# nathancunn/ParticleMDI.jl

Hardware: NVIDIA B200
Metric: particle*cluster*feature evals/sec (dense count P*N*sum_k D_k per observation step) (higher is better)
Workload: dtype f64

## Files before the change

particlemdi.jl_b200/csrc/pmdi_cuda.cu:

```cuda
#include "../../include/pmdi_cuda.h"

#include <cuda_runtime.h>
#include <dlfcn.h>

#include <algorithm>
#include <chrono>
#include <cmath>
#include <cstdio>
#include <cstring>
#include <cstdlib>
#include <map>
#include <queue>
#include <string>
#include <vector>

#include "aux_kernels.cuh"
#include "sweep_kernel.cuh"
#include "pool_kernel.cuh"
#include "spec_kernel.cuh"
#include "summary_kernels.cuh"

#include "pmdi_embedded.inc"

#ifndef __CUDA_ARCH__
// ... 61 lines not shown

struct Dataset {
  bool bound = false;
  int type = -1, D = 0, Dp = 0, J = 0, Lmax = 0, FB = PMDI_FB;
  int user = -1, uW = 0;
  int slot = 0;
  DevBuf<double> ust;
  long long max_arg = 0;
  std::vector<uint8_t> flag;
  std::vector<double> nlevels;
  bool rc_dirty = true;
  DevBuf<unsigned char> x, xq;
  bool xq_dirty = true;
  DevBuf<uint8_t> d_flag;
  DevBuf<double> rc, d_nlevels;
  DevBuf<double> mu, lamn, sum, beta, part, aux;
  DevBuf<uint32_t> cnt;
  DevBuf<long long> S;
  DevBuf<int> n;
  int cap = 0, wpf = 1, fpw = 4;
  DevBuf<unsigned long long> cw;
  DevBuf<int> p_refcnt, p_chosen, p_dst, p_neval, p_live, p_free, p_rowmap, p_ctr;
  DevBuf<double> p_lp;
  DevBuf<RowInfo> p_info;
  DevBuf<int> p_mark;
  void release() {
    x.release(); xq.release(); d_flag.release(); rc.release(); d_nlevels.release();
    mu.release(); lamn.release(); sum.release(); beta.release(); part.release(); aux.release();
    cnt.release(); S.release(); n.release(); cw.release(); ust.release();
    p_refcnt.release(); p_chosen.release(); p_dst.release(); p_neval.release(); p_live.release();
    p_free.release(); p_rowmap.release(); p_ctr.release(); p_lp.release();
    p_info.release(); p_mark.release();
  }
};

}

struct pmdi_ctx {
  int K = 0, N = 0, P = 0, device = 0;
  long long n = 0;
  cudaStream_t stream = nullptr;
  bool own_stream = false;
  int n_sm = 0, G = 0, GP = 0;
  int sm_budget = 0;
  pmdi_group* group = nullptr;
  std::vector<Dataset> ds;
  bool layout_dirty = true;
  unsigned char* arena = nullptr;
  size_t arena_bytes = 0;
  int rank = 0, R = 1, Ps = 0;
  int engine = 1;
  int engine_req = PMDI_ENGINE_AUTO;
  int obs_ring = PMDI_OBS_RING;
  unsigned long long wd_ns = 10000000000ull;
  long long peer_delta[8] = {0, 0, 0, 0, 0, 0, 0, 0};
  void* peer_base[8] = {nullptr, nullptr, nullptr, nullptr, nullptr, nullptr, nullptr, nullptr};
  std::vector<int> cta_off, cta_units;
  int max_units = 0, sm_x_bytes = 0, lf_T = 0, lf_want = 0, item_cap = 0, Jmax = 0;
  bool assigned = false;
  size_t dyn_smem = 0;
  std::vector<double> lf_host;
  DevBuf<double> lf_dev;
  DevBuf<int> d_cta_off, d_cta_units;
  DevBuf<double> Pi, l1phi, tape_alloc, tape_resamp, tape_shuffle, tape_select;
  DevBuf<long long> s_in, s_out, d_pstar, cluster_n, counters;
  DevBuf<int> order, slot_of, anc_log, ev_of_step, members, mem_off, cur_at, plan_out, err;
  DevBuf<int> sc_j, sc_anc0, sc_a, sc_b, sc_c, sc_d;
  DevBuf<double> lw, lw_out, sc_w, sc_pp, sc_u, inc, lp_empty, ess_part;
  DevBuf<int> logical_of;
  DevBuf<uint8_t> lab, alloc_log;
  DevBuf<int2> copies;
  DevBuf<unsigned> bar;
  DevBuf<unsigned long long> rows_eval, rows_ref, phase_ns, trace;
  DevBuf<long long> label_counts, pair_agree, contingency;
  DevBuf<unsigned> psm;
  DevBuf<long long> psm_s;
  long long psm_samples = 0;
  DevBuf<double> rank_part;
  DevBuf<int4> pull_jobs;
  DevBuf<int> pull_map;
  bool pull_map_init = false;
  DevBuf<unsigned char> dec;
  DevBuf<int4> glist, elist;
  DevBuf<int> gcnt;
  DevBuf<unsigned long long> rows_spec, rows_add;
  DevBuf<double> dbg_lp, dbg_lw, scratch_d;
  DevBuf<int> dbg_alloc, dbg_anc, scratch_i, wd_state;
  DevBuf<uint8_t> scratch_u8;
  SweepParams sp;
  bool uploaded = false, ran = false;
  cudaLibrary_t jit_lib = nullptr;
  std::string jit_key;
  std::vector<UserType> jit_types;
  bool has_user = false;
  unsigned step_seq = 0;
  unsigned long long sweep_seq = 1;
  DevBuf<unsigned long long> bar_state;
  bool bar_state_init = false;
  unsigned sweep_flags = 0;
  cudaEvent_t ev0 = nullptr, ev1 = nullptr, ev2 = nullptr, ev3 = nullptr;
  DevBuf<unsigned char> inblk, outblk;
  unsigned char *h_in = nullptr, *h_out = nullptr;
  size_t in_bytes = 0, out_bytes = 0, out_head = 0;
  struct { size_t s_in, Pi, l1phi, order; } ioff;
  struct { size_t err, counters, rows_eval, rows_ref, rows_spec, rows_add, pstar, label_counts, pair_agree,
           contingency, lw_out, s_out, phase, cluster_n; } ooff;
  cudaEvent_t ev_h2d = nullptr;
};

namespace {

int round_up(int v, int m) { return (v + m - 1) / m * m; }

void fill_dsdev(pmdi_ctx* c, int k, DsDev& d) {
  Dataset& s = c->ds[k];
  std::memset(&d, 0, sizeof(d));
  d.type = s.type; d.D = s.D; d.Dp = s.Dp; d.J = s.J; d.Lmax = s.type == T_USER ? s.slot : s.Lmax; d.FB = s.FB;
  int nflag = 0;
  for (int q = 0; q < s.D; ++q) nflag += s.flag[q] ? 1 : 0;
  d.nflag = nflag;
  d.all_on = (nflag == s.D && s.D == s.Dp) ? 1 : 0;
  if (s.type == T_GAUSSIAN && nflag == s.D) d.all_on = 1;
  d.x = s.x.p; d.flag = s.d_flag.p; d.rc = s.rc.p;
  d.xstage = (s.type != T_GAUSSIAN && s.type != T_USER && nflag != s.D) ? (const void*)s.xq.p : (const void*)s.x.p;
  d.mu = s.mu.p; d.lamn = s.lamn.p; d.sum = s.sum.p; d.beta = s.beta.p;
  d.uW = s.type == T_USER ? (user_types()[s.user].elem_kind == PMDI_F64 ? s.uW : -s.uW) : 0;
  d.ust = s.ust.p;
  d.cnt = s.cnt.p; d.S = s.S.p; d.part = c->engine ? nullptr : s.part.p; d.aux = s.aux.p; d.n = s.n.p;
}

void fill_pooldev(pmdi_ctx* c, int k, PoolDev& d) {
  Dataset& s = c->ds[k];
  std::memset(&d, 0, sizeof(d));
  d.cap = s.cap; d.wpf = s.wpf; d.fpw = s.fpw;
  d.refcnt = s.p_refcnt.p; d.chosen = s.p_chosen.p; d.dst = s.p_dst.p; d.n_eval = s.p_neval.p;
  d.live = s.p_live.p; d.freelist = s.p_free.p; d.rowmap = s.p_rowmap.p; d.ctr = s.p_ctr.p; d.cw = s.cw.p;
  d.lp = s.p_lp.p; d.info = s.p_info.p; d.mark = s.p_mark.p;
}

int build_rc(pmdi_ctx* c, int k) {
  Dataset& s = c->ds[k];
  const long long n = c->n;
  std::vector<double> rc(n + 1);
  int nflag = 0;
  for (int q = 0; q < s.D; ++q) nflag += s.flag[q] ? 1 : 0;
  if (s.type == T_USER) {
    std::fill(rc.begin(), rc.end(), 0.0);
  } else if (s.type == T_GAUSSIAN) {
    for (long long i = 0; i <= n; ++i) {
      const double nn = (double)i;
      rc[i] = nflag * (std::log(1.0 / std::sqrt(M_PI)) + std::lgamma(0.5 * nn + 1.0) -
                       std::lgamma(0.5 * nn + 0.5));
    }
  } else if (s.type == T_CATEGORICAL) {
    std::map<double, long long> hist;
    for (int q = 0; q < s.D; ++q)
      if (s.flag[q]) hist[s.nlevels[q]] += 1;
    for (long long i = 0; i <= n; ++i) {
      double acc = 0.0;
      for (auto& kv : hist) acc += (double)kv.second * std::log(kv.first + (double)i);
      rc[i] = -acc;
    }
  } else {
    for (long long i = 0; i <= n; ++i) rc[i] = nflag * std::log((double)i + 1.0);
  }
  CK(s.rc.ensure(n + 1));
// ... 467 lines not shown
  if (tag == PMDI_ALL_USER_TYPES) {
    for (int u = 0; u < (int)user_types().size(); ++u) users.push_back(u);
    if (users.empty()) return fail(1, "pmdi_cluster_type_check: no cluster type registered");
  } else {
    const int user = tag - USER_TAG0;
    if (user < 0 || user >= (int)user_types().size()) return fail(1, "pmdi_cluster_type_check: unknown type tag");
    users.push_back(user);
  }
  const char* eng = getenv("PMDI_ENGINE");
  const std::string* cubin = nullptr;
  return jit_compile(registered(users), eng && std::string(eng) == "spec" ? 2 : 1, cubin);
}

int pmdi_group_type_check(const int32_t* tags, int32_t n) {
  if (!tags) return fail(1, "pmdi_group_type_check: tags is NULL");
  if (n < 1 || n > PMDI_MAX_K) return fail(1, "pmdi_group_type_check: need 1 <= n <= 8 cluster types");
  std::vector<int> users;
  for (int i = 0; i < n; ++i) {
    const int user = tags[i] - USER_TAG0;
    if (user < 0 || user >= (int)user_types().size())
      return fail(1, "pmdi_group_type_check: tags[" + std::to_string(i) + "] is not a registered user type");
    users.push_back(user);
  }
  const std::string* cubin = nullptr;
  return jit_compile(registered(users), JIT_SPEC_GROUP, cubin);
}

int pmdi_ctx_create(pmdi_ctx** out, int32_t K, int64_t n_obs, int32_t N, int32_t particles,
                    int32_t device) {
  if (!out) return fail(1, "pmdi_ctx_create: out is NULL");
  *out = nullptr;
  if (K < 1 || K > PMDI_MAX_K) return fail(1, "pmdi_ctx_create: need 1 <= K <= 8 datasets");
  if (!(N > 1 && (int64_t)N <= n_obs)) return fail(1, "pmdi_ctx_create: need 1 < N <= n_obs");
  if (N > PMDI_MAX_N) return fail(1, "pmdi_ctx_create: N > 256 is not supported");
  if (particles <= 1) return fail(1, "pmdi_ctx_create: need particles > 1");
  if (n_obs > 0x7fffffff / 2) return fail(1, "pmdi_ctx_create: n_obs too large");
  if (pmdi_device_count() <= device || device < 0)
    return fail(2, "pmdi_ctx_create: no CUDA device " + std::to_string(device) +
                       " (libpmdi_cuda has no CPU fallback)");
  CK(cudaSetDevice(device));
  cudaDeviceProp prop;
  CK(cudaGetDeviceProperties(&prop, device));
  if (prop.major < 10)
    return fail(2, "pmdi_ctx_create: built for sm_100a (B200); found compute capability " +
                       std::to_string(prop.major) + "." + std::to_string(prop.minor));
  int coop = 0;
  CK(cudaDeviceGetAttribute(&coop, cudaDevAttrCooperativeLaunch, device));
  if (!coop) return fail(2, "pmdi_ctx_create: device lacks cooperative launch");
  pmdi_ctx* c = new pmdi_ctx();
  c->K = K; c->n = n_obs; c->N = N; c->P = particles; c->device = device;
  c->n_sm = prop.multiProcessorCount;
  c->G = c->n_sm;
  c->sm_budget = c->n_sm;
  c->ds.resize(K);
  std::memset(&c->sp, 0, sizeof(c->sp));
  cudaError_t e = cudaStreamCreateWithFlags(&c->stream, cudaStreamNonBlocking);
  if (e != cudaSuccess) { delete c; return fail(100 + (int)e, "cudaStreamCreate failed"); }
  c->own_stream = true;
  cudaEventCreate(&c->ev0); cudaEventCreate(&c->ev1); cudaEventCreate(&c->ev2); cudaEventCreate(&c->ev3);
  *out = c;
  return 0;
}

static void group_detach(pmdi_ctx* c);

int pmdi_ctx_destroy(pmdi_ctx* c) {
  if (!c) return 0;
  cudaSetDevice(c->device);
  if (c->group) group_detach(c);
  cudaStreamSynchronize(c->stream);
  for (auto& d : c->ds) d.release();
  DevBuf<double>* dd[] = {&c->lf_dev, &c->Pi, &c->l1phi, &c->tape_alloc, &c->tape_resamp, &c->tape_shuffle,
                          &c->tape_select, &c->lw, &c->lw_out, &c->sc_w, &c->sc_pp, &c->sc_u, &c->dbg_lp,
                          &c->dbg_lw, &c->scratch_d, &c->inc, &c->lp_empty, &c->ess_part};
  for (auto* b : dd) b->release();
  DevBuf<int>* di[] = {&c->d_cta_off, &c->d_cta_units, &c->order, &c->slot_of, &c->anc_log, &c->ev_of_step,
                       &c->members, &c->mem_off, &c->cur_at, &c->plan_out, &c->err, &c->sc_j, &c->sc_anc0,
                       &c->sc_a, &c->sc_b, &c->sc_c, &c->sc_d, &c->dbg_alloc, &c->dbg_anc, &c->scratch_i, &c->logical_of};
  for (auto* b : di) b->release();
  DevBuf<long long>* dl[] = {&c->s_in, &c->s_out, &c->d_pstar, &c->cluster_n, &c->counters};
  for (auto* b : dl) b->release();
  c->lab.release(); c->alloc_log.release(); c->copies.release(); c->bar.release();
  c->rows_eval.release(); c->phase_ns.release(); c->scratch_u8.release();
  c->dec.release(); c->rows_spec.release(); c->rows_add.release(); c->bar_state.release(); c->glist.release(); c->elist.release(); c->gcnt.release();
  c->rows_ref.release(); c->trace.release(); c->wd_state.release(); c->pull_jobs.release(); c->pull_map.release(); c->rank_part.release();
  c->label_counts.release(); c->pair_agree.release(); c->contingency.release(); c->psm.release(); c->psm_s.release();
  for (int r = 0; r < c->R; ++r)
    if (r != c->rank && c->peer_base[r]) cudaIpcCloseMemHandle(c->peer_base[r]);
  c->inblk.release(); c->outblk.release();
  if (c->h_in) cudaFreeHost(c->h_in);
  if (c->h_out) cudaFreeHost(c->h_out);
  if (c->ev_h2d) cudaEventDestroy(c->ev_h2d);
  if (c->arena) cudaFree(c->arena);
  if (c->jit_lib) cudaLibraryUnload(c->jit_lib);
  if (c->ev0) { cudaEventDestroy(c->ev0); cudaEventDestroy(c->ev1); cudaEventDestroy(c->ev2); cudaEventDestroy(c->ev3); }
  if (c->own_stream && c->stream) cudaStreamDestroy(c->stream);
  delete c;
  return 0;
}

int pmdi_ctx_set_engine(pmdi_ctx* c, int32_t engine) {
  if (!c) return fail(1, "pmdi_ctx_set_engine: NULL context");
  if (engine != PMDI_ENGINE_AUTO && engine != PMDI_ENGINE_POOL && engine != PMDI_ENGINE_SPEC)
    return fail(1, "pmdi_ctx_set_engine: engine is PMDI_ENGINE_AUTO (-1), PMDI_ENGINE_POOL (1) or PMDI_ENGINE_SPEC (2)");
  if (c->arena)
    return fail(1, "pmdi_ctx_set_engine: the context has already been prepared for the " + engine_name(c->engine) +
                       " engine (first upload, sweep, feature or cluster-eval call), and its memory layout depends on "
                       "the engine: choose the engine before that");
  c->engine_req = engine;
  return 0;
}

int pmdi_ctx_set_stream(pmdi_ctx* c, void* s) {
  if (!c) return fail(1, "NULL context");
  if (c->own_stream && c->stream) cudaStreamDestroy(c->stream);
  c->stream = (cudaStream_t)s;
  c->own_stream = false;
  return 0;
}
void* pmdi_ctx_get_stream(pmdi_ctx* c) { return c ? (void*)c->stream : nullptr; }

int pmdi_set_dataset(pmdi_ctx* c, int32_t k, int32_t type_tag, int32_t elem_kind, const void* data,
                     int64_t n_obs, int64_t D, int64_t ld) {
  if (!c) return fail(1, "NULL context");
  if (k < 0 || k >= c->K) return fail(1, "pmdi_set_dataset: k out of range");
  if (n_obs != c->n) return fail(1, "pmdi_set_dataset: datasets must have n_obs rows (src/pmdi.jl:52)");
  if (D < 1 || D > 8192) return fail(1, "pmdi_set_dataset: need 1 <= D <= 8192 features per dataset");
  if (ld < n_obs) return fail(1, "pmdi_set_dataset: ld < n_obs");
  const int user = type_tag >= USER_TAG0 ? type_tag - USER_TAG0 : -1;
  if (user >= (int)user_types().size() || (user < 0 && (type_tag < 0 || type_tag > 2)))
    return fail(1, "pmdi_set_dataset: unknown cluster type tag");
  if (user >= 0) {
    if (elem_kind != user_types()[user].elem_kind)
      return fail(1, "pmdi_set_dataset: cluster type '" + user_types()[user].name + "' was registered for the other element kind");
  } else if ((type_tag == PMDI_GAUSSIAN) != (elem_kind == PMDI_F64)) {
    return fail(1, "pmdi_set_dataset: Gaussian needs PMDI_F64 data, Categorical/NegBinom need PMDI_I64");
  }
  CK(cudaSetDevice(c->device));
  Dataset& s = c->ds[k];
  s.release();
  s.type = user >= 0 ? T_USER : type_tag; s.user = user; s.D = (int)D; s.Dp = round_up((int)D, PMDI_WF);
  s.J = (s.Dp + PMDI_FB - 1) / PMDI_FB;
  s.Lmax = 0; s.max_arg = 0;
  const long long n = c->n;
  const int Dp = s.Dp;
  s.flag.assign(Dp, 0);
  for (int q = 0; q < s.D; ++q) s.flag[q] = 1;
  if (user >= 0) {
    const int w = user_words_guess(user_types()[user].src);
    if (w < 1 || w > 8) return fail(1, "pmdi_set_dataset: the user type needs `static constexpr int WORDS = 1..8;`");
    s.uW = w;
  }
  if (elem_kind == PMDI_F64) {
    std::vector<double> h((size_t)n * Dp, 0.0);
    const double* x = (const double*)data;
    for (int q = 0; q < s.D; ++q)
      for (long long i = 0; i < n; ++i) h[(size_t)i * Dp + q] = x[(size_t)i + (size_t)ld * q];
    CK(s.x.ensure(h.size() * 8));
    CK(cudaMemcpy(s.x.p, h.data(), h.size() * 8, cudaMemcpyHostToDevice));
  } else {
    std::vector<int> h((size_t)n * Dp, (type_tag == PMDI_NEGBINOM) ? -1 : 0);
    const int64_t* x = (const int64_t*)data;
    s.nlevels.assign(s.D, 0.0);
    long long gmax = 0, max_colsum = 0;
    for (int q = 0; q < s.D; ++q) {
      long long cmax = x[(size_t)ld * q], csum = 0;
      for (long long i = 0; i < n; ++i) {
// ... 171 lines not shown
    if (o != c->out_bytes) {
      CK(cudaStreamSynchronize(st));
      if (c->h_out) cudaFreeHost(c->h_out);
      CK(cudaHostAlloc((void**)&c->h_out, o, cudaHostAllocDefault));
      CK(c->outblk.ensure(o));
      c->out_bytes = o; c->out_head = head;
    }
    unsigned char* b = c->outblk.p;
    c->err.view(b + c->ooff.err, 4); c->counters.view(b + c->ooff.counters, 8);
    c->rows_eval.view(b + c->ooff.rows_eval, PMDI_MAX_K); c->rows_ref.view(b + c->ooff.rows_ref, PMDI_MAX_K);
    c->rows_spec.view(b + c->ooff.rows_spec, PMDI_MAX_K); c->rows_add.view(b + c->ooff.rows_add, PMDI_MAX_K);
    c->d_pstar.view(b + c->ooff.pstar, 1); c->label_counts.view(b + c->ooff.label_counts, (size_t)N * K);
    c->pair_agree.view(b + c->ooff.pair_agree, std::max(npairs, 1));
    c->contingency.view(b + c->ooff.contingency, (size_t)std::max(npairs, 1) * N * N);
    c->lw_out.view(b + c->ooff.lw_out, P); c->s_out.view(b + c->ooff.s_out, n * K);
    c->phase_ns.view(b + c->ooff.phase, 8 * (size_t)c->G); c->cluster_n.view(b + c->ooff.cluster_n, (size_t)K * P * N);
  }
  CK(cudaEventSynchronize(c->ev_h2d));
  {
    int* order = (int*)(c->h_in + c->ioff.order);
    std::vector<uint8_t> seen(n, 0);
    for (long long i = 0; i < n; ++i) {
      const int64_t o = a->order_obs[i];
      if (o < 1 || o > n || seen[o - 1]) return fail(1, "pmdi_sweep: order_obs is not a permutation of 1..n_obs");
      seen[o - 1] = 1;
      order[i] = (int)(o - 1);
    }
    for (long long i = 0; i < n * K; ++i)
      if (a->s[i] < 1 || a->s[i] > N) return fail(1, "pmdi_sweep: allocation label outside 1..N");
    std::memcpy(c->h_in + c->ioff.s_in, a->s, sizeof(int64_t) * n * K);
    std::memcpy(c->h_in + c->ioff.Pi, a->Pi, sizeof(double) * N * K);
    double* l1phi = (double*)(c->h_in + c->ioff.l1phi);
    for (int i = 0; i < npairs; ++i) l1phi[i] = std::log(1 + a->phi[i]);
    CK(cudaMemcpyAsync(c->inblk.p, c->h_in, c->in_bytes, cudaMemcpyHostToDevice, st));
    CK(cudaEventRecord(c->ev_h2d, st));
  }
  sp.tape_alloc = sp.tape_resamp = sp.tape_shuffle = sp.tape_select = nullptr;
  if (a->tape_alloc) {
    CK(c->tape_alloc.ensure((size_t)steps * K * P));
    CK(cudaMemcpyAsync(c->tape_alloc.p, a->tape_alloc, sizeof(double) * steps * K * P, cudaMemcpyHostToDevice, st));
    sp.tape_alloc = c->tape_alloc.p;
  }
  if (a->tape_resamp) {
    CK(c->tape_resamp.ensure(steps));
    CK(cudaMemcpyAsync(c->tape_resamp.p, a->tape_resamp, sizeof(double) * steps, cudaMemcpyHostToDevice, st));
    sp.tape_resamp = c->tape_resamp.p;
  }
  if (a->tape_shuffle) {
    CK(c->tape_shuffle.ensure((size_t)steps * P));
    CK(cudaMemcpyAsync(c->tape_shuffle.p, a->tape_shuffle, sizeof(double) * steps * P, cudaMemcpyHostToDevice, st));
    sp.tape_shuffle = c->tape_shuffle.p;
  }
  if (a->tape_select) {
    CK(c->tape_select.ensure(1));
    CK(cudaMemcpyAsync(c->tape_select.p, a->tape_select, sizeof(double), cudaMemcpyHostToDevice, st));
    sp.tape_select = c->tape_select.p;
  }
  CK(c->lw_out.ensure(P)); CK(c->slot_of.ensure(2 * (size_t)P));
  CK(c->logical_of.ensure(2 * (size_t)P)); CK(c->inc.ensure(2 * (size_t)K * P)); CK(c->lp_empty.ensure((size_t)steps * K));
  CK(c->lab.ensure(2 * (size_t)K * P));
  CK(c->anc_log.ensure((size_t)steps * P)); CK(c->ev_of_step.ensure(steps));
  CK(c->sc_w.ensure(P)); CK(c->sc_pp.ensure(P)); CK(c->sc_u.ensure(P));
  CK(c->sc_j.ensure(P)); CK(c->sc_anc0.ensure(P)); CK(c->sc_a.ensure(P)); CK(c->sc_b.ensure(P));
  CK(c->sc_c.ensure(P)); CK(c->sc_d.ensure(P)); CK(c->copies.ensure(P)); CK(c->plan_out.ensure(4));
  CK(c->err.ensure(4)); CK(c->rows_eval.ensure(PMDI_MAX_K)); CK(c->counters.ensure(8));
  CK(c->phase_ns.ensure(8 * (size_t)c->G)); CK(c->d_pstar.ensure(1)); CK(c->cluster_n.ensure((size_t)K * P * N));
  CK(c->members.ensure((size_t)K * std::max<long long>(a->n1 - 1, 1))); CK(c->mem_off.ensure((size_t)K * (N + 1)));
  CK(c->cur_at.ensure(steps));
  CK(c->rows_ref.ensure(PMDI_MAX_K)); CK(c->label_counts.ensure((size_t)N * K)); CK(c->pair_agree.ensure(std::max(npairs, 1)));
  CK(c->contingency.ensure((size_t)std::max(npairs, 1) * N * N));
  sp.rows_ref = c->rows_ref.p;
  CK(c->dec.ensure(steps)); CK(c->rows_spec.ensure(PMDI_MAX_K)); CK(c->rows_add.ensure(PMDI_MAX_K));
  CK(cudaMemsetAsync(c->rows_spec.p, 0, 8 * PMDI_MAX_K, st));
  CK(cudaMemsetAsync(c->rows_add.p, 0, 8 * PMDI_MAX_K, st));
  sp.dec = c->dec.p; sp.rows_spec = c->rows_spec.p; sp.rows_add = c->rows_add.p;
  if (c->engine == 2) {
    const long long lcap = (long long)K * ((long long)c->Ps * N + N + 2);
    CK(c->glist.ensure(lcap)); CK(c->gcnt.ensure(4));
    CK(c->elist.ensure(2 * (size_t)(c->G - c->GP - 1) * lcap));
    CK(cudaMemsetAsync(c->gcnt.p, 0, 16, st));
    sp.glist = c->glist.p; sp.gcnt = c->gcnt.p; sp.elist = c->elist.p; sp.lcap = lcap;
    const long long cap = c->ds[0].cap, ge = c->G - c->GP - 1;
    sp.fc_target = (int)std::max<long long>(8, std::min<long long>(SPEC_FC / 2, cap / (4 * ge)));
    sp.plan_smem = (size_t)32 * P + 64 <= c->dyn_smem ? 1 : 0;
  }
  sp.pull_jobs = nullptr;
  if (c->engine && c->R > 1) {
    CK(c->pull_jobs.ensure(2 * (size_t)K * c->Ps * N));
    sp.pull_jobs = c->pull_jobs.p;
    if (c->engine == 2) {
      const size_t n_map = (size_t)K * c->R * c->ds[0].cap;
      CK(c->pull_map.ensure(n_map));
      if (!c->pull_map_init) { CK(cudaMemsetAsync(c->pull_map.p, 0xff, sizeof(int) * n_map, st)); c->pull_map_init = true; }
      sp.pull_map = c->pull_map.p;
    }
  }
  sp.n1 = (int)a->n1; sp.steps = steps; sp.flags = (int)a->flags;
  sp.Pi = c->Pi.p; sp.l1phi = c->l1phi.p; sp.s_in = c->s_in.p; sp.order = c->order.p;
  sp.lw_init = a->logweight_init; sp.seed = a->seed; sp.iter = a->iter;
  sp.lw = c->lw.p; sp.ess_part = c->ess_part.p; sp.lw_out = c->lw_out.p; sp.slot_of = c->slot_of.p; sp.logical_of = c->logical_of.p;
  sp.inc = c->inc.p; sp.lp_empty = c->lp_empty.p; sp.lab = c->lab.p;
  sp.alloc_log = c->alloc_log.p + (c->sweep_seq & 1) * (size_t)n * K * P;
  sp.tag_base = c->sweep_seq << 32;
  sp.tag32 = c->step_seq;
  CK(c->bar_state.ensure(2));
  if (!c->bar_state_init) { CK(cudaMemsetAsync(c->bar_state.p, 0, 16, st)); c->bar_state_init = true; }
  sp.bar_state = c->bar_state.p;
  sp.anc_log = c->anc_log.p; sp.ev_of_step = c->ev_of_step.p;
  sp.sc_w = c->sc_w.p; sp.sc_pp = c->sc_pp.p; sp.sc_u = c->sc_u.p; sp.sc_j = c->sc_j.p;
  sp.sc_anc0 = c->sc_anc0.p; sp.sc_a = c->sc_a.p; sp.sc_b = c->sc_b.p; sp.sc_c = c->sc_c.p;
  sp.sc_d = c->sc_d.p; sp.copies = c->copies.p; sp.plan_out = c->plan_out.p;
  sp.bar = c->bar.p; sp.err = c->err.p; sp.rows_eval = c->rows_eval.p; sp.counters = c->counters.p;
  sp.phase_ns = (a->flags & PMDI_SWEEP_TIME_PHASES) ? c->phase_ns.p : nullptr;
  sp.dbg_lp = nullptr; sp.dbg_lw = nullptr; sp.dbg_alloc = nullptr; sp.dbg_anc = nullptr;
  if (a->flags & PMDI_SWEEP_DEBUG) {
    CK(c->dbg_lp.ensure((size_t)steps * K * P * N)); CK(c->dbg_lw.ensure((size_t)steps * P));
    CK(c->dbg_alloc.ensure((size_t)steps * K * P)); CK(c->dbg_anc.ensure((size_t)steps * P));
    CK(cudaMemsetAsync(c->dbg_anc.p, 0, sizeof(int) * (size_t)steps * P, st));
    CK(cudaMemsetAsync(c->dbg_lp.p, 0, sizeof(double) * (size_t)steps * K * P * N, st));
    CK(cudaMemsetAsync(c->dbg_lw.p, 0, sizeof(double) * (size_t)steps * P, st));
    CK(cudaMemsetAsync(c->dbg_alloc.p, 0, sizeof(int) * (size_t)steps * K * P, st));
    sp.dbg_lp = c->dbg_lp.p; sp.dbg_lw = c->dbg_lw.p; sp.dbg_alloc = c->dbg_alloc.p; sp.dbg_anc = c->dbg_anc.p;
  }
  if (c->R > 1 && c->peer_base[c->rank] == nullptr)
    return fail(1, "pmdi_sweep: call pmdi_ipc_export / pmdi_ipc_import on every rank first");
  if (!c->engine) {
    CK(cudaMemsetAsync(c->bar.p, 0, 16, st));
  }
  CK(cudaMemsetAsync(c->phase_ns.p, 0, 64 * (size_t)c->G, st));
  CK(c->wd_state.ensure((size_t)c->G * 16 * 16));
  CK(cudaMemsetAsync(c->wd_state.p, 0xff, sizeof(int) * (size_t)c->G * 16 * 16, st));
  sp.wd_state = c->wd_state.p;
  sp.trace = nullptr;
  if (getenv("PMDI_TRACE_STEP")) {
    CK(c->trace.ensure(16 * 128));
    CK(cudaMemsetAsync(c->trace.p, 0, 16 * 128 * 8, st));
    sp.trace = c->trace.p;
    sp.trace_step = atoi(getenv("PMDI_TRACE_STEP"));
    sp.trace_cta = getenv("PMDI_TRACE_CTA") ? atoi(getenv("PMDI_TRACE_CTA")) : 0;
  }
  c->sweep_flags = a->flags;
  c->uploaded = true;
  c->ran = false;
  if (!c->engine && c->R > 1) CK(cudaStreamSynchronize(st));
  return 0;
}

}

namespace {

int queue_setup(pmdi_ctx* c, cudaStream_t st) {
  const SweepParams& sp = c->sp;
  const int K = c->K, N = c->N, P = c->P;
  CK(cudaEventRecord(c->ev0, st));
  k_sweep_init<<<(P + 255) / 256, 256, 0, st>>>(sp);
  if (sp.n1 > 1) {
    k_prefix_lists<<<K, PMDI_MAX_N + 32, 0, st>>>(sp, c->members.p, c->mem_off.p);
  } else {
    CK(cudaMemsetAsync(c->mem_off.p, 0, sizeof(int) * K * (N + 1), st));
  }
  int maxDp = 0;
  for (int k = 0; k < K; ++k) maxDp = std::max(maxDp, c->ds[k].Dp);
  KFN(fn_build, c, k_prefix_build)
  CK(launch_on(st, fn_build, dim3((maxDp + 127) / 128, N, K), dim3(128), 0, sp, (const int*)c->members.p,
               (const int*)c->mem_off.p));
// ... 933 lines not shown
```

particlemdi.jl_b200/csrc/pmdi_internal.h:

```cpp
#ifndef PMDI_INTERNAL_H
#define PMDI_INTERNAL_H
#ifdef __CUDACC_RTC__
typedef unsigned char uint8_t;
typedef int int32_t;
typedef unsigned int uint32_t;
typedef long long int64_t;
typedef unsigned long long uint64_t;
#else
#include <stdint.h>
#endif

#define PMDI_MAX_K 8
#define PMDI_MAX_N 256
#define PMDI_FB 256
#define PMDI_WF 64
#define PMDI_NT 512
#define PMDI_OBS_RING 4

enum { T_GAUSSIAN = 0, T_CATEGORICAL = 1, T_NEGBINOM = 2, T_USER = 3  };
enum { DRAW_ALLOC = 0, DRAW_RESAMP = 1, DRAW_SHUFFLE = 2, DRAW_SELECT = 3, DRAW_FEATURE = 4 };

#define PMDI_XBYTES(ds_) (((ds_).type == T_GAUSSIAN || ((ds_).type == T_USER && (ds_).uW > 0)) ? 8u : 4u)

struct DsDev {
// ... 31 lines not shown
  int* freelist;
  int* rowmap;
  int* ctr;
  unsigned long long* cw;
  double* lp;
  RowInfo* info;
  int* mark;
};

struct __attribute__((aligned(16))) SweepParams {
  int K, N, P, n_obs, n1, steps;
  int G, flags;
  int R, rank, Ps, slot0;
  long long peer_delta[8];
  DsDev ds[PMDI_MAX_K];
  PoolDev pd[PMDI_MAX_K];
  int engine;
  int GP;
  unsigned char* dec;
  unsigned long long* rows_spec;
  int4* glist;
  int* gcnt;
  int4* elist;
  long long lcap;
  int fc_target;
  int plan_smem;
  int pad1;
  unsigned long long* rows_add;
  unsigned long long tag_base;
  unsigned long long* bar_state;
  int obs_ring;
  long long proto_base;
  unsigned long long wd_ns;
  int4* pull_jobs;
  int* pull_map;
  double* rank_part;
  unsigned long long* rank_words;
  unsigned tag32;
  unsigned long long* rows_ref;
  const double* Pi;
  const double* l1phi;
  const long long* s_in;
  const int* order;
  double lw_init;
  unsigned long long seed;
  unsigned iter;
  int Jmax;
  const double *tape_alloc, *tape_resamp, *tape_shuffle, *tape_select;
  double* lw;
  double* ess_part;
  double* lw_out;
  int* slot_of;
  int* logical_of;
  uint8_t* lab;
  double* inc;
  const double* lp_empty;
  uint8_t* alloc_log;
  int* anc_log;
  int* ev_of_step;
  double *sc_w, *sc_pp, *sc_u;
  int *sc_j, *sc_anc0, *sc_a, *sc_b, *sc_c, *sc_d;
  int2* copies;
  int* plan_out;
  const int* cta_off;
  const int* cta_units;
  int max_units, sm_x_bytes;
  int lf_T, item_cap;
  int qb;
  int jq;
  const double* lf_glob;
  int lf_glob_T;
  unsigned* bar;
  int* err;
  unsigned long long* rows_eval;
  long long* counters;
  unsigned long long* phase_ns;
  unsigned long long* trace;
  int trace_cta, trace_step;
  int* wd_state;
  double* dbg_lp;
  double* dbg_lw;
  int* dbg_alloc;
  int* dbg_anc;
};

#endif
```

particlemdi.jl_b200/csrc/spec_kernel.cuh:

```cuda
#pragma once
#include "pool_types.cuh"
#include "sweep_common.cuh"

#define SPEC_FC 256
#define SPEC_EC 512

struct SpecSmem {
  unsigned long long obs_bar[PMDI_OBS_RING];
  unsigned long long epoch, xepoch;
  double res_mx;
  double red[2][2][64];
  int res_flag;
  int fail;
  int ev;
  int pdone;
  int lpar;
  int cnt;
  int wsum[PMDI_NW];
  int b_tt[PMDI_MAX_K], b_c[PMDI_MAX_K], b_cc[PMDI_MAX_K], b_next[PMDI_MAX_K];
  int kc[PMDI_MAX_K];
  unsigned kadd[PMDI_MAX_K];
  unsigned rows_eval[PMDI_MAX_K], rows_ref[PMDI_MAX_K], rows_spec[PMDI_MAX_K];
  unsigned long long tacc[8];
  int tr_n[PMDI_NW];
// ... 605 lines not shown
      }
      if (lane == 0) atomicAdd(&sm.rows_spec[k], mode ? 2u : 1u);
    }
    SWEEP_TRACE(st - 1, 66)
  }
  if (t_dec >= 0 && threadIdx.x == 32) {
    int d;
    const unsigned long long t0 = globaltimer_ns();
    unsigned spins = 0;
#pragma unroll 1
    while ((d = *(volatile unsigned char*)(sp.dec + t_dec)) == 0) {
      if (((++spins) & 0x3ffu) == 0 && (__ldcg(sp.err) != 0 || globaltimer_ns() - t0 > sp.wd_ns)) {
        atomicCAS(sp.err, 0, 77); sm.fail = 1; break;
      }
    }
    sm.res_flag = d == 2;
  }
  __syncthreads();
}

#define SPEC_PULL_PARTS 16
__device__ __noinline__ void spec_row_pull(const SweepParams& sp, int4 j0, int4 j1, int parn, int part) {
  const int k = j0.x & 0xff, ra = j0.x >> 8, rb = j0.y, v2 = j0.z, c2 = j0.w, a2 = j1.x, b2 = j1.y;
  const DsDev& ds = sp.ds[k];
  const PoolDev& pd = sp.pd[k];
  const long long sdelta = sp.peer_delta[ra];
  const int lane = threadIdx.x & 31, Dp = ds.Dp;
#define PMDI_SRC(ptr_) ((decltype(ptr_))((const char*)(ptr_) + sdelta))
  const RowInfo* rinfo = PMDI_SRC(pd.info);
  const int4 i1 = ldcg_info(rinfo + (size_t)parn * pd.cap + rb);
  const int rc = i1.z;
  const int4 i2 = ldcg_info(rinfo + (size_t)(parn ^ 1) * pd.cap + rb);
  const int4 i2c = ldcg_info(rinfo + (size_t)(parn ^ 1) * pd.cap + rc);
  const int n = ldcg_i32(PMDI_SRC(ds.n) + rb);
  long long W = ds.type == T_CATEGORICAL ? (long long)Dp * pd.wpf : (long long)Dp;
#ifdef PMDI_USER_TYPES
  if (ds.type == T_USER) W = user_row_words(ds);
#endif
  const long long per = ((W / 64 + SPEC_PULL_PARTS - 1) / SPEC_PULL_PARTS) * 64;
  const long long q_lo = part * per, q_hi = min(W, q_lo + per);
#pragma unroll 1
  for (int h = 0; h < 2; ++h) {
    const long long src = h ? rc : rb, dst = h ? c2 : v2;
    if (ds.type == T_GAUSSIAN) {
#pragma unroll 1
      for (long long q = q_lo + 2 * lane; q < q_hi; q += 64) {
        const double2 a = ldcg_f64x2(PMDI_SRC(ds.mu) + src * Dp + q), b = ldcg_f64x2(PMDI_SRC(ds.lamn) + src * Dp + q);
        const double2 c = ldcg_f64x2(PMDI_SRC(ds.sum) + src * Dp + q), d = ldcg_f64x2(PMDI_SRC(ds.beta) + src * Dp + q);
        *(double2*)(ds.mu + dst * Dp + q) = a; *(double2*)(ds.lamn + dst * Dp + q) = b;
        *(double2*)(ds.sum + dst * Dp + q) = c; *(double2*)(ds.beta + dst * Dp + q) = d;
      }
    } else if (ds.type == T_CATEGORICAL) {
#pragma unroll 1
      for (long long q = q_lo + 2 * lane; q < q_hi; q += 64)
        *(ulonglong2*)(pd.cw + dst * W + q) = ldcg_u64x2(PMDI_SRC(pd.cw) + src * W + q);
#ifdef PMDI_USER_TYPES
    } else if (ds.type == T_USER) {
#pragma unroll 1
      for (long long q = q_lo + 2 * lane; q < q_hi; q += 64)
        *(double2*)(ds.ust + dst * W + q) = ldcg_f64x2(PMDI_SRC(ds.ust) + src * W + q);
#endif
    } else {
#pragma unroll 1
      for (long long q = q_lo + 2 * lane; q < q_hi; q += 64)
        *(longlong2*)(ds.S + dst * Dp + q) = ldcg_i64x2(PMDI_SRC(ds.S) + src * Dp + q);
    }
    if (part == 0) {
#pragma unroll 1
      for (int jj = lane; jj < ds.J; jj += 32) ds.aux[dst * ds.J + jj] = ldcg_f64(PMDI_SRC(ds.aux) + src * ds.J + jj);
    }
  }
#undef PMDI_SRC
  if (lane == 0 && part == 0) {
    ds.n[v2] = n; ds.n[c2] = n + 1; ds.n[a2] = n + 1; ds.n[b2] = n + 2;
    int4 w = i1; w.z = c2; w.w = 0;
    *(int4*)(pd.info + (size_t)parn * pd.cap + v2) = w;
    w = i2; w.z = a2; w.w = 0;
    *(int4*)(pd.info + (size_t)(parn ^ 1) * pd.cap + v2) = w;
    w = i2c; w.z = b2; w.w = 0;
    *(int4*)(pd.info + (size_t)(parn ^ 1) * pd.cap + c2) = w;
  }
}

template <bool GRP>
__device__ __noinline__ bool spec_resample(const SweepParams& sp, SpecSmem& sm, const SpecTables& T, int ns, int st,
                                           int* s_tmp, bool is_p, int e) {
  const int K = sp.K, N = sp.N, Ps = sp.Ps;
  const int ev = sm.ev;
  const long long gt = (long long)spec_cta<GRP>() * PMDI_NT + threadIdx.x, GT = (long long)sp.G * PMDI_NT;
  const int parn = (st + 1) & 1;
  const bool has_next = st + 1 < sp.steps;
  const bool tm = sp.phase_ns != nullptr && threadIdx.x == 0;
  unsigned long long t_ = tm ? globaltimer_ns() : 0ull;
#define RS_MARK(i_) if (tm) { const unsigned long long n_ = globaltimer_ns(); sm.tacc[i_] += (n_ - t_) * PMDI_NW; t_ = n_; }
  if (!spec_xsync(sp, sm)) return false;
  if (spec_cta<GRP>() == sp.G - 1) {
    extern __shared__ __align__(16) unsigned char plan_raw[];
    PlanScratch sc = {sp.sc_w, sp.sc_pp, sp.sc_u, sp.sc_j, sp.sc_anc0};
    if (sp.plan_smem) {
      sc.w = (double*)plan_raw; sc.pp = sc.w + sp.P; sc.u = sc.pp + sp.P;
      sc.j = (int*)(sc.u + sp.P); sc.a0 = sc.j + sp.P;
    }
    pool_resample_plan(sp, st, ev, sm.res_mx, s_tmp, sp.lw + (size_t)(st & 1) * sp.P, sc);
  }
  if (!spec_gsync(sp, sm)) return false;
  RS_MARK(4)
  const int* anc = sp.anc_log + (size_t)ev * sp.P;
  if (gt == (long long)sp.GP * PMDI_NT && has_next)
    atomicAdd((unsigned long long*)&sp.counters[4], (unsigned long long)sm.cnt);
#pragma unroll 1
  for (int k = 0; k < K; ++k) {
    const PoolDev& pd = sp.pd[k];
    const int* rm_old = pd.rowmap + (size_t)(ev & 1) * Ps * N;
    int* rm_new = pd.rowmap + (size_t)((ev + 1) & 1) * Ps * N;
#pragma unroll 1
    for (long long i = gt; i < (long long)Ps * N; i += GT) {
      const int slot = (int)(i / N), m = (int)(i - (long long)slot * N);
      const int a = ldcg_i32(anc + sp.slot0 + slot) - 1;
      const int ra = a / Ps, la = a - ra * Ps;
      if (ra == sp.rank) {
        __stcg(rm_new + i, ldcg_i32(rm_old + (size_t)la * N + m));
      } else if (slot == 0 || ldcg_i32(anc + sp.slot0 + slot - 1) != a + 1) {
        const int rb = ldcg_i32(on_rank(sp, rm_old, ra) + (size_t)la * N + m);
        if (rb != pd.cap - 1) {
          int* pm = sp.pull_map + ((size_t)k * sp.R + ra) * pd.cap + rb;
          if (atomicCAS(pm, -1, -2) == -1) {
            const int first = atomicSub(pd.ctr + 1, 4) - 4;
            if (first < 0) { atomicExch(sp.err, 80); sm.fail = 1; }
            else {
              const int v2 = spec_gtake(pd, first), c2 = spec_gtake(pd, first + 1);
              const int a2 = spec_gtake(pd, first + 2), b2 = spec_gtake(pd, first + 3);
              const long long job = atomicAdd((unsigned long long*)&sp.counters[5], 1ull);
              sp.pull_jobs[2 * job] = make_int4(k | (ra << 8), rb, v2, c2);
              sp.pull_jobs[2 * job + 1] = make_int4(a2, b2, 0, 0);
              __stcg(pm, v2);
            }
          }
        }
      }
    }
  }
  if (sp.R > 1) {
    if (!spec_gsync(sp, sm)) return false;
#pragma unroll 1
    for (int k = 0; k < K; ++k) {
      const PoolDev& pd = sp.pd[k];
      const int* rm_old = pd.rowmap + (size_t)(ev & 1) * Ps * N;
      int* rm_new = pd.rowmap + (size_t)((ev + 1) & 1) * Ps * N;
#pragma unroll 1
      for (long long i = gt; i < (long long)Ps * N; i += GT) {
        const int slot = (int)(i / N), m = (int)(i - (long long)slot * N);
        const int a = ldcg_i32(anc + sp.slot0 + slot) - 1;
        const int ra = a / Ps, la = a - ra * Ps;
        if (ra == sp.rank || !(slot == 0 || ldcg_i32(anc + sp.slot0 + slot - 1) != a + 1)) continue;
        const int rb = ldcg_i32(on_rank(sp, rm_old, ra) + (size_t)la * N + m);
        __stcg(rm_new + i, rb == pd.cap - 1 ? rb : ldcg_i32(sp.pull_map + ((size_t)k * sp.R + ra) * pd.cap + rb));
      }
    }
    if (!spec_gsync(sp, sm)) return false;
    const long long njobs = __ldcg(&sp.counters[5]);
    const long long gw = gt >> 5, GWp = GT >> 5;
#pragma unroll 1
    for (long long item = gw; item < njobs * SPEC_PULL_PARTS; item += GWp) {
      const long long job = item / SPEC_PULL_PARTS;
      const int part = (int)(item - job * SPEC_PULL_PARTS);
      const int4 j0 = __ldcg(sp.pull_jobs + 2 * job);
      spec_row_pull(sp, j0, __ldcg(sp.pull_jobs + 2 * job + 1), parn, part);
      if (part == 0 && (threadIdx.x & 31) == 0)
        __stcg(sp.pull_map + ((size_t)(j0.x & 0xff) * sp.R + (j0.x >> 8)) * sp.pd[j0.x & 0xff].cap + j0.y, -1);
    }
    if (gt == 0) sp.counters[3] += njobs;
#pragma unroll 1
    for (int k = 0; k < K; ++k) {
      int* rm_new = sp.pd[k].rowmap + (size_t)((ev + 1) & 1) * Ps * N;
#pragma unroll 1
      for (long long i = gt; i < (long long)Ps * N; i += GT) {
        const int slot = (int)(i / N), m = (int)(i - (long long)slot * N);
        const int a1 = ldcg_i32(anc + sp.slot0 + slot);
        if ((a1 - 1) / Ps == sp.rank) continue;
        int f = slot;
        while (f > 0 && ldcg_i32(anc + sp.slot0 + f - 1) == a1) --f;
        if (f != slot) __stcg(rm_new + i, ldcg_i32(rm_new + (size_t)f * N + m));
      }
    }
    if (!spec_gsync(sp, sm)) return false;
    if (gt == 0) sp.counters[5] = 0;
  }
  RS_MARK(5)
#pragma unroll 1
  for (int k = 0; k < K; ++k) {
    const PoolDev& pd = sp.pd[k];
    int* rc_new = pd.refcnt + (size_t)parn * pd.cap;
#pragma unroll 1
    for (long long r = gt; r < pd.cap; r += GT) {
      __stcg(rc_new + r, 0); __stcg(pd.mark + r, 0); __stcg(pd.freelist + r, -1);
      __stcg(pd.chosen + r, 0); __stcg(pd.chosen + pd.cap + r, 0); __stcg(pd.chosen + 2 * (size_t)pd.cap + r, 0);
    }
  }
  if (is_p)
    for (int sl = threadIdx.x; sl < ns; sl += PMDI_NT) T.lw_s[sl] = 1.0;
  if (!spec_gsync(sp, sm)) return false;
#pragma unroll 1
  for (int k = 0; k < K; ++k) {
    const PoolDev& pd = sp.pd[k];
    const int* rm_new = pd.rowmap + (size_t)((ev + 1) & 1) * Ps * N;
    int* rc_new = pd.refcnt + (size_t)parn * pd.cap;
#pragma unroll 1
    for (long long i = gt; i < (long long)Ps * N; i += GT) atomicAdd(rc_new + ldcg_i32(rm_new + i), 1);
  }
  if (gt == 0) {
    *sp.gcnt = 0;
    for (int k = 0; k < K; ++k) __stcg(sp.pd[k].ctr + 1, 0);
  }
  if (!spec_gsync(sp, sm)) return false;
#pragma unroll 1
  for (int k = 0; k < K; ++k) {
    const PoolDev& pd = sp.pd[k];
    const int empty = pd.cap - 1;
    const int* rc_new = pd.refcnt + (size_t)parn * pd.cap;
#pragma unroll 1
    for (long long r = gt; r < pd.cap; r += GT) {
      if (r != empty && ldcg_i32(rc_new + r) == 0) continue;
      if (!has_next) continue;
      const int c = ldcg_info(pd.info + (size_t)parn * pd.cap + r).z;
      __stcg(pd.mark + c, 1);
      __stcg(pd.mark + ldcg_info(pd.info + (size_t)(parn ^ 1) * pd.cap + r).z, 1);
      __stcg(pd.mark + ldcg_info(pd.info + (size_t)(parn ^ 1) * pd.cap + c).z, 1);
    }
  }
  if (!spec_gsync(sp, sm)) return false;
#pragma unroll 1
  for (int k = 0; k < K; ++k) {
    const PoolDev& pd = sp.pd[k];
    const int* rc_new = pd.refcnt + (size_t)parn * pd.cap;
#pragma unroll 1
    for (long long rb = (gt >> 5) << 5; rb < pd.cap - 1; rb += GT) {
      const long long r = rb + (threadIdx.x & 31);
      const bool in = r < pd.cap - 1;
      const int rc = in ? ldcg_i32(rc_new + r) : 1;
      if (in && rc > 0) {
        const int i = atomicAdd(sp.gcnt, 1);
        const int c = has_next ? ldcg_info(pd.info + (size_t)parn * pd.cap + r).z : -1;
        __stcg(sp.glist + i, make_int4((k << SPEC_KSHIFT) | (int)r, c, ldcg_i32(sp.ds[k].n + r), 0));
      }
      const bool fr = in && rc == 0 && !ldcg_i32(pd.mark + r);
      const unsigned m = __ballot_sync(FULL, fr);
      if (m) {
        int base = 0;
        const int leader = __ffs(m) - 1;
        if ((int)(threadIdx.x & 31) == leader) base = atomicAdd(pd.ctr + 1, __popc(m));
        base = __shfl_sync(FULL, base, leader);
        if (fr) pd.freelist[base + __popc(m & ((1u << (threadIdx.x & 31)) - 1u))] = (int)r;
      }
    }
  }
  if (!spec_xsync(sp, sm)) return false;
  RS_MARK(7)
#undef RS_MARK
  if (gt == 0 && has_next) atomicAdd((unsigned long long*)&sp.counters[4], (unsigned long long)(-(long long)ldcg_i32(sp.gcnt)));
  if (threadIdx.x == 0) { sm.ev = ev + 1; sm.res_flag = 0; }
  __syncthreads();
  if (is_p) {
    spec_load_units<GRP>(sp, sm, T, ns);
  } else if (e >= 0) {
    const int nl = ldcg_i32(sp.gcnt);
#pragma unroll 1
    for (int i = threadIdx.x; i < nl; i += PMDI_NT) spec_set_entry(sp, T, e, 0, i, __ldcg(sp.glist + i));
    if (threadIdx.x < K) { T.fc_top[threadIdx.x] = 0; sm.kc[threadIdx.x] = 0; }
    if (threadIdx.x == 0) { sm.cnt = nl; sm.lpar = 0; }
    if (has_next) spec_load_empty_next(sp, sm, parn);
  }
  __syncthreads();
  return !sm.fail;
}

template <bool DBG, bool GRP>
__device__ __forceinline__ void spec_sweep_body(const SweepParams& sp, SpecSmem& sm, unsigned char* smem_raw, int* s_tmp) {
  const int tid = threadIdx.x, lane = tid & 31, warp = tid >> 5;
  const int NW = PMDI_NW;
  const int cta = spec_cta<GRP>();
  const int K = sp.K, N = sp.N, steps = sp.steps, GP = sp.GP;
  const bool is_p = cta < GP;
  const int e = cta - GP;
  const int Npad = (N + 31) & ~31;
  const int ns = is_p ? (sp.Ps - cta + GP - 1) / GP : 0;
  const int nu = ns * K;
  const int MS = (sp.Ps + GP - 1) / GP, MU = MS * K;

  unsigned char* xring = smem_raw;
  SpecTables T;
  T.lf = (double*)(smem_raw + (size_t)sp.obs_ring * sp.sm_x_bytes);
  unsigned char* rt = (unsigned char*)(T.lf + ((sp.lf_T + 1) & ~1));
  T.lp_s = (double*)rt;
  T.Pi_s = T.lp_s + (size_t)NW * Npad;
  T.lw_s = T.Pi_s + (size_t)K * N;
  T.inc_s = T.lw_s + MS;
  T.lw_prev = T.inc_s + MU;
  T.ch_s = (int*)(T.lw_prev + MS);
  T.lab_s = T.ch_s + (size_t)NW * Npad;
  T.pcount = T.lab_s + MU;
  T.u_c = T.pcount + MS;
  T.u_child = T.u_c + MU;
  T.u_occ = T.u_child + MU;
  T.u_c1 = T.u_occ + MU;
  T.u_c2 = T.u_c1 + MU;
  T.u_prow = T.u_c2 + MU;
  T.u_ks = T.u_prow + MU;
  T.rm_s = T.u_ks + MU;
  T.el_s = (int4*)rt;
  T.fc_s = (int*)(T.el_s + (size_t)2 * SPEC_EC);
  T.fc_top = T.fc_s + (size_t)K * SPEC_FC;
  if (tid < PMDI_MAX_K) { sm.rows_eval[tid] = 0; sm.rows_ref[tid] = 0; sm.rows_spec[tid] = 0; sm.kadd[tid] = 0; }
  if (tid < 8) sm.tacc[tid] = 0;
  if (tid < PMDI_NW) sm.tr_n[tid] = 0;
  if (tid == 0) {
    sm.res_flag = 0; sm.fail = 0; sm.ev = 0; sm.pdone = 0; sm.res_mx = 0.0;
    sm.epoch = __ldcg(sp.bar_state); sm.xepoch = __ldcg(sp.bar_state + 1);
    sm.lpar = 0; sm.cnt = 0;
    for (int b = 0; b < sp.obs_ring; ++b) mbar_init(&sm.obs_bar[b], 1);
    asm volatile("fence.mbarrier_init.release.cluster;" ::: "memory");
  }
  __syncthreads();
  if (is_p) {
#pragma unroll 1
    for (int i = tid; i < K * N; i += PMDI_NT) T.Pi_s[i] = sp.Pi[i];
#pragma unroll 1
    for (int sl = tid; sl < ns; sl += PMDI_NT) { T.lw_s[sl] = sp.lw_init; T.pcount[sl] = 0; }
#pragma unroll 1
    for (int u = tid; u < nu; u += PMDI_NT) T.u_ks[u] = (u % K) | ((u / K) << 8);
    spec_load_units<GRP>(sp, sm, T, ns);
  } else if (cta != sp.G - 1) {
    if (tid == 0)
      for (int s = 0; s < sp.obs_ring; ++s) pool_issue_obs(sp, s, xring, sm.obs_bar);
#pragma unroll 1
    for (int i = tid; i < sp.lf_T; i += PMDI_NT) T.lf[i] = sp.lf_glob[i];
    const int nl = ldcg_i32(sp.gcnt);
#pragma unroll 1
    for (int i = tid; i < nl; i += PMDI_NT) spec_set_entry(sp, T, e, 0, i, __ldcg(sp.glist + i));
    if (tid < K) { T.fc_top[tid] = 0; sm.kc[tid] = 0; }
    if (tid == 0) sm.cnt = nl;
    __syncthreads();
    if (e == 0)
      for (int i = tid; i < nl; i += PMDI_NT) atomicAdd(&sm.kc[(unsigned)spec_entry(sp, T, e, 0, i).x >> SPEC_KSHIFT], 1);
    spec_refill(sp, sm, T);
  }
  __syncthreads();

  const bool timing = DBG && sp.phase_ns != nullptr;
  unsigned long long tw_prev = timing ? globaltimer_ns() : 0ull;
#define PHASE_MARK(i_)                                                 \
  if (DBG && timing && lane == 0) {                                    \
// ... 185 lines not shown
```

Before: 1389 billion.

## Fuse resample refcount/mark passes and deal free rows directly to CTAs

Moves the clearing of refcount, mark, freelist and chosen arrays into the planning phase run by non-planner CTAs. Refcount accumulation and next-step marking are folded into the rowmap-copy loop using warp match_any aggregation. This removes two grid-wide syncs and several full passes over the pool. Freed rows are also dealt straight into a per-CTA deal buffer that each CTA loads into its shared free cache, with only the overflow going to the global freelist. The cost is added complexity in counter handling (ctr+2 versus ctr+1) and a separate path for multi-rank runs.

```diff
diff --git a/particlemdi.jl_b200/csrc/pmdi_cuda.cu b/particlemdi.jl_b200/csrc/pmdi_cuda.cu
--- a/particlemdi.jl_b200/csrc/pmdi_cuda.cu
+++ b/particlemdi.jl_b200/csrc/pmdi_cuda.cu
@@ -167,6 +167,7 @@
   bool pull_map_init = false;
   DevBuf<unsigned char> dec;
   DevBuf<int4> glist, elist;
+  DevBuf<int> deal;
   DevBuf<int> gcnt;
   DevBuf<unsigned long long> rows_spec, rows_add;
   DevBuf<double> dbg_lp, dbg_lw, scratch_d;
@@ -800,7 +801,7 @@
   for (auto* b : dl) b->release();
   c->lab.release(); c->alloc_log.release(); c->copies.release(); c->bar.release();
   c->rows_eval.release(); c->phase_ns.release(); c->scratch_u8.release();
-  c->dec.release(); c->rows_spec.release(); c->rows_add.release(); c->bar_state.release(); c->glist.release(); c->elist.release(); c->gcnt.release();
+  c->dec.release(); c->rows_spec.release(); c->rows_add.release(); c->bar_state.release(); c->glist.release(); c->elist.release(); c->gcnt.release(); c->deal.release();
   c->rows_ref.release(); c->trace.release(); c->wd_state.release(); c->pull_jobs.release(); c->pull_map.release(); c->rank_part.release();
   c->label_counts.release(); c->pair_agree.release(); c->contingency.release(); c->psm.release(); c->psm_s.release();
   for (int r = 0; r < c->R; ++r)
@@ -1138,6 +1139,8 @@
     sp.glist = c->glist.p; sp.gcnt = c->gcnt.p; sp.elist = c->elist.p; sp.lcap = lcap;
     const long long cap = c->ds[0].cap, ge = c->G - c->GP - 1;
     sp.fc_target = (int)std::max<long long>(8, std::min<long long>(SPEC_FC / 2, cap / (4 * ge)));
+    CK(c->deal.ensure((size_t)K * ge * sp.fc_target));
+    sp.deal = c->deal.p;
     sp.plan_smem = (size_t)32 * P + 64 <= c->dyn_smem ? 1 : 0;
   }
   sp.pull_jobs = nullptr;
diff --git a/particlemdi.jl_b200/csrc/pmdi_internal.h b/particlemdi.jl_b200/csrc/pmdi_internal.h
--- a/particlemdi.jl_b200/csrc/pmdi_internal.h
+++ b/particlemdi.jl_b200/csrc/pmdi_internal.h
@@ -137,6 +137,7 @@
   double* dbg_lw;
   int* dbg_alloc;
   int* dbg_anc;
+  int* deal;
 };
 
 #endif
diff --git a/particlemdi.jl_b200/csrc/spec_kernel.cuh b/particlemdi.jl_b200/csrc/spec_kernel.cuh
--- a/particlemdi.jl_b200/csrc/spec_kernel.cuh
+++ b/particlemdi.jl_b200/csrc/spec_kernel.cuh
@@ -711,6 +711,20 @@
   }
 }
 
+__device__ __forceinline__ void spec_mark_next(const PoolDev& pd, int parn, int r) {
+  const int c = ldcg_info(pd.info + (size_t)parn * pd.cap + r).z;
+  __stcg(pd.mark + c, 1);
+  __stcg(pd.mark + ldcg_info(pd.info + (size_t)(parn ^ 1) * pd.cap + r).z, 1);
+  __stcg(pd.mark + ldcg_info(pd.info + (size_t)(parn ^ 1) * pd.cap + c).z, 1);
+}
+__device__ __forceinline__ void spec_count_ref(const PoolDev& pd, int* rc_new, int r, int parn, bool has_next) {
+  const unsigned g = __match_any_sync(FULL, r);
+  if (r >= 0 && (int)(threadIdx.x & 31) == __ffs(g) - 1) {
+    atomicAdd(rc_new + r, __popc(g));
+    if (has_next) spec_mark_next(pd, parn, r);
+  }
+}
+
 template <bool GRP>
 __device__ __noinline__ bool spec_resample(const SweepParams& sp, SpecSmem& sm, const SpecTables& T, int ns, int st,
                                            int* s_tmp, bool is_p, int e) {
@@ -731,6 +745,28 @@
       sc.j = (int*)(sc.u + sp.P); sc.a0 = sc.j + sp.P;
     }
     pool_resample_plan(sp, st, ev, sm.res_mx, s_tmp, sp.lw + (size_t)(st & 1) * sp.P, sc);
+  } else {
+    const long long GT1 = GT - PMDI_NT;
+#pragma unroll 1
+    for (int k = 0; k < K; ++k) {
+      const PoolDev& pd = sp.pd[k];
+      int* rc_new = pd.refcnt + (size_t)parn * pd.cap;
+#pragma unroll 1
+      for (long long r = gt; r < pd.cap; r += GT1) {
+        __stcg(rc_new + r, 0); __stcg(pd.mark + r, 0);
+        if (sp.R == 1) __stcg(pd.freelist + r, -1);
+        __stcg(pd.chosen + r, 0); __stcg(pd.chosen + pd.cap + r, 0); __stcg(pd.chosen + 2 * (size_t)pd.cap + r, 0);
+      }
+    }
+    if (gt == 0) {
+      *sp.gcnt = 0;
+      for (int k = 0; k < K; ++k) {
+        __stcg(sp.pd[k].ctr + 2, 0);
+        if (sp.R == 1) __stcg(sp.pd[k].ctr + 1, 0);
+      }
+    }
+    if (is_p)
+      for (int sl = threadIdx.x; sl < ns; sl += PMDI_NT) T.lw_s[sl] = 1.0;
   }
   if (!spec_gsync(sp, sm)) return false;
   RS_MARK(4)
@@ -742,31 +778,39 @@
     const PoolDev& pd = sp.pd[k];
     const int* rm_old = pd.rowmap + (size_t)(ev & 1) * Ps * N;
     int* rm_new = pd.rowmap + (size_t)((ev + 1) & 1) * Ps * N;
-#pragma unroll 1
-    for (long long i = gt; i < (long long)Ps * N; i += GT) {
-      const int slot = (int)(i / N), m = (int)(i - (long long)slot * N);
-      const int a = ldcg_i32(anc + sp.slot0 + slot) - 1;
-      const int ra = a / Ps, la = a - ra * Ps;
-      if (ra == sp.rank) {
-        __stcg(rm_new + i, ldcg_i32(rm_old + (size_t)la * N + m));
-      } else if (slot == 0 || ldcg_i32(anc + sp.slot0 + slot - 1) != a + 1) {
-        const int rb = ldcg_i32(on_rank(sp, rm_old, ra) + (size_t)la * N + m);
-        if (rb != pd.cap - 1) {
-          int* pm = sp.pull_map + ((size_t)k * sp.R + ra) * pd.cap + rb;
-          if (atomicCAS(pm, -1, -2) == -1) {
-            const int first = atomicSub(pd.ctr + 1, 4) - 4;
-            if (first < 0) { atomicExch(sp.err, 80); sm.fail = 1; }
-            else {
-              const int v2 = spec_gtake(pd, first), c2 = spec_gtake(pd, first + 1);
-              const int a2 = spec_gtake(pd, first + 2), b2 = spec_gtake(pd, first + 3);
-              const long long job = atomicAdd((unsigned long long*)&sp.counters[5], 1ull);
-              sp.pull_jobs[2 * job] = make_int4(k | (ra << 8), rb, v2, c2);
-              sp.pull_jobs[2 * job + 1] = make_int4(a2, b2, 0, 0);
-              __stcg(pm, v2);
+    int* rc_new = pd.refcnt + (size_t)parn * pd.cap;
+    if (gt == 0 && has_next) spec_mark_next(pd, parn, pd.cap - 1);
+#pragma unroll 1
+    for (long long i0 = gt & ~31ll; i0 < (long long)Ps * N; i0 += GT) {
+      const long long i = i0 + (threadIdx.x & 31);
+      int row = -1;
+      if (i < (long long)Ps * N) {
+        const int slot = (int)(i / N), m = (int)(i - (long long)slot * N);
+        const int a = ldcg_i32(anc + sp.slot0 + slot) - 1;
+        const int ra = a / Ps, la = a - ra * Ps;
+        if (ra == sp.rank) {
+          row = ldcg_i32(rm_old + (size_t)la * N + m);
+          __stcg(rm_new + i, row);
+        } else if (slot == 0 || ldcg_i32(anc + sp.slot0 + slot - 1) != a + 1) {
+          const int rb = ldcg_i32(on_rank(sp, rm_old, ra) + (size_t)la * N + m);
+          if (rb != pd.cap - 1) {
+            int* pm = sp.pull_map + ((size_t)k * sp.R + ra) * pd.cap + rb;
+            if (atomicCAS(pm, -1, -2) == -1) {
+              const int first = atomicSub(pd.ctr + 1, 4) - 4;
+              if (first < 0) { atomicExch(sp.err, 80); sm.fail = 1; }
+              else {
+                const int v2 = spec_gtake(pd, first), c2 = spec_gtake(pd, first + 1);
+                const int a2 = spec_gtake(pd, first + 2), b2 = spec_gtake(pd, first + 3);
+                const long long job = atomicAdd((unsigned long long*)&sp.counters[5], 1ull);
+                sp.pull_jobs[2 * job] = make_int4(k | (ra << 8), rb, v2, c2);
+                sp.pull_jobs[2 * job + 1] = make_int4(a2, b2, 0, 0);
+                __stcg(pm, v2);
+              }
             }
           }
         }
       }
+      if (sp.R == 1) spec_count_ref(pd, rc_new, row, parn, has_next);
     }
   }
   if (sp.R > 1) {
@@ -814,54 +858,29 @@
     }
     if (!spec_gsync(sp, sm)) return false;
     if (gt == 0) sp.counters[5] = 0;
-  }
+#pragma unroll 1
+    for (int k = 0; k < K; ++k) {
+      const PoolDev& pd = sp.pd[k];
+      const int* rm_new = pd.rowmap + (size_t)((ev + 1) & 1) * Ps * N;
+      int* rc_new = pd.refcnt + (size_t)parn * pd.cap;
+#pragma unroll 1
+      for (long long r = gt; r < pd.cap; r += GT) __stcg(pd.freelist + r, -1);
+      if (gt == 0) __stcg(pd.ctr + 1, 0);
+#pragma unroll 1
+      for (long long i0 = gt & ~31ll; i0 < (long long)Ps * N; i0 += GT) {
+        const long long i = i0 + (threadIdx.x & 31);
+        spec_count_ref(pd, rc_new, i < (long long)Ps * N ? ldcg_i32(rm_new + i) : -1, parn, has_next);
+      }
+    }
+  }
+  if (!spec_gsync(sp, sm)) return false;
   RS_MARK(5)
-#pragma unroll 1
-  for (int k = 0; k < K; ++k) {
-    const PoolDev& pd = sp.pd[k];
-    int* rc_new = pd.refcnt + (size_t)parn * pd.cap;
-#pragma unroll 1
-    for (long long r = gt; r < pd.cap; r += GT) {
-      __stcg(rc_new + r, 0); __stcg(pd.mark + r, 0); __stcg(pd.freelist + r, -1);
-      __stcg(pd.chosen + r, 0); __stcg(pd.chosen + pd.cap + r, 0); __stcg(pd.chosen + 2 * (size_t)pd.cap + r, 0);
-    }
-  }
-  if (is_p)
-    for (int sl = threadIdx.x; sl < ns; sl += PMDI_NT) T.lw_s[sl] = 1.0;
-  if (!spec_gsync(sp, sm)) return false;
-#pragma unroll 1
-  for (int k = 0; k < K; ++k) {
-    const PoolDev& pd = sp.pd[k];
-    const int* rm_new = pd.rowmap + (size_t)((ev + 1) & 1) * Ps * N;
-    int* rc_new = pd.refcnt + (size_t)parn * pd.cap;
-#pragma unroll 1
-    for (long long i = gt; i < (long long)Ps * N; i += GT) atomicAdd(rc_new + ldcg_i32(rm_new + i), 1);
-  }
-  if (gt == 0) {
-    *sp.gcnt = 0;
-    for (int k = 0; k < K; ++k) __stcg(sp.pd[k].ctr + 1, 0);
-  }
-  if (!spec_gsync(sp, sm)) return false;
-#pragma unroll 1
-  for (int k = 0; k < K; ++k) {
-    const PoolDev& pd = sp.pd[k];
-    const int empty = pd.cap - 1;
-    const int* rc_new = pd.refcnt + (size_t)parn * pd.cap;
-#pragma unroll 1
-    for (long long r = gt; r < pd.cap; r += GT) {
-      if (r != empty && ldcg_i32(rc_new + r) == 0) continue;
-      if (!has_next) continue;
-      const int c = ldcg_info(pd.info + (size_t)parn * pd.cap + r).z;
-      __stcg(pd.mark + c, 1);
-      __stcg(pd.mark + ldcg_info(pd.info + (size_t)(parn ^ 1) * pd.cap + r).z, 1);
-      __stcg(pd.mark + ldcg_info(pd.info + (size_t)(parn ^ 1) * pd.cap + c).z, 1);
-    }
-  }
-  if (!spec_gsync(sp, sm)) return false;
+  const int n_deal = (sp.G - sp.GP - 1) * sp.fc_target;
 #pragma unroll 1
   for (int k = 0; k < K; ++k) {
     const PoolDev& pd = sp.pd[k];
     const int* rc_new = pd.refcnt + (size_t)parn * pd.cap;
+    int* deal = sp.deal + (size_t)k * n_deal;
 #pragma unroll 1
     for (long long rb = (gt >> 5) << 5; rb < pd.cap - 1; rb += GT) {
       const long long r = rb + (threadIdx.x & 31);
@@ -877,9 +896,16 @@
       if (m) {
         int base = 0;
         const int leader = __ffs(m) - 1;
-        if ((int)(threadIdx.x & 31) == leader) base = atomicAdd(pd.ctr + 1, __popc(m));
+        if ((int)(threadIdx.x & 31) == leader) {
+          base = atomicAdd(pd.ctr + 2, __popc(m));
+          if (base + __popc(m) > n_deal) atomicMax(pd.ctr + 1, base + __popc(m) - n_deal);
+        }
         base = __shfl_sync(FULL, base, leader);
-        if (fr) pd.freelist[base + __popc(m & ((1u << (threadIdx.x & 31)) - 1u))] = (int)r;
+        const int pos = base + __popc(m & ((1u << (threadIdx.x & 31)) - 1u));
+        if (fr) {
+          if (pos < n_deal) __stcg(deal + pos, (int)r);
+          else pd.freelist[pos - n_deal] = (int)r;
+        }
       }
     }
   }
@@ -895,7 +921,16 @@
     const int nl = ldcg_i32(sp.gcnt);
 #pragma unroll 1
     for (int i = threadIdx.x; i < nl; i += PMDI_NT) spec_set_entry(sp, T, e, 0, i, __ldcg(sp.glist + i));
-    if (threadIdx.x < K) { T.fc_top[threadIdx.x] = 0; sm.kc[threadIdx.x] = 0; }
+    const int tgt = sp.fc_target;
+#pragma unroll 1
+    for (int i = threadIdx.x; i < K * tgt; i += PMDI_NT) {
+      const int k = i / tgt, j = i - k * tgt, pos = e * tgt + j;
+      if (pos < ldcg_i32(sp.pd[k].ctr + 2)) T.fc_s[k * SPEC_FC + j] = __ldcg(sp.deal + (size_t)k * n_deal + pos);
+    }
+    if (threadIdx.x < K) {
+      T.fc_top[threadIdx.x] = min(tgt, max(0, ldcg_i32(sp.pd[threadIdx.x].ctr + 2) - e * tgt));
+      sm.kc[threadIdx.x] = 0;
+    }
     if (threadIdx.x == 0) { sm.cnt = nl; sm.lpar = 0; }
     if (has_next) spec_load_empty_next(sp, sm, parn);
   }
```

Result: faster. 1426 billion (median of 6 runs) (+2.6%).
